# TropComplique/MultiPoseNet

Measured on AMD Instinct MI355X. Metric: images/sec keypoint fwd+bwd+Adam @512x512 bs32/GPU, higher is better.
Workload: dtype bf16; 1 GPU; MobileNet-v1+FPN+keypoint_subnet fwd+bwd+Adam, 512x512, per-GPU batch 32; global_batch=32, parallelism=dp1, hip_graph=True, rccl_ranks=1

## Files before the change

include/mpn.h:

```cpp
#ifndef MPN_H_
#define MPN_H_

#include <stddef.h>
#include <stdint.h>

#ifdef __cplusplus
extern "C" {
#endif

#define MPN_VERSION 600

enum { MPN_F32 = 0, MPN_BF16 = 1, MPN_F16 = 2  };

enum {
    MPN_OK = 0,
    MPN_ERR_BAD_SHAPE = -1,
    MPN_ERR_BAD_DTYPE = -2,
    MPN_ERR_BAD_ALIGN = -3,
    MPN_ERR_HIP = -4,
    MPN_ERR_BAD_ARG = -5,
    MPN_ERR_WORKSPACE = -6,
    MPN_ERR_BAD_DATA = -7
};

// ... 34 lines not shown
                         const float* bn_shift, int bn_act, float* part, mpn_stream_t stream);
int mpn_conv_bwd_data_bn_grouped(int njobs, const void* const* dy, const void* const* w_packed_t, void* const* dx, int N,
                                 const int* H, const int* W, int K, int C, const int* dy_stride, const int* dx_stride,
                                 int dtype, const void* const* bn_x, const int* bn_x_stride, const float* const* bn_scale,
                                 const float* const* bn_shift, int bn_act, float* const* part, mpn_stream_t stream);

int mpn_conv_wgrad_num_parts(int N, int H, int W, int Cin, int Cout, int ksize, int dtype);
int mpn_conv_bwd_weight(const void* x, const void* dy, float* part, int N, int H, int W, int Cin,
                        int Cout, int x_stride, int dy_stride, int ksize, int dtype, const float* in_scale,
                        const float* in_shift, int in_act, mpn_stream_t stream);

int mpn_conv1x1_bwd_fused_supported(int Cin, int Cout, int dtype);
int mpn_conv1x1_bwd_fused(const void* x, const void* dy, const float* w, void* dx, float* wpart, float* bn_part, int N, int H, int W,
                          int Cin, int Cout, int x_stride, int dy_stride, int dx_stride, int dtype, const float* in_scale,
                          const float* in_shift, int in_act, mpn_stream_t stream);
int mpn_conv1x1_bwd_fused_apply_supported(int Cin, int Cout, int dtype);
int mpn_conv1x1_bwd_fused_apply(const void* x, const void* g, const void* y_raw, const float* w, void* dx, float* wpart, float* bn_part,
                                int N, int H, int W, int Cin, int Cout, int x_stride, int g_stride, int y_stride, int dx_stride,
                                int dtype, const float* in_scale, const float* in_shift, int in_act, const float* ap_scale,
                                const float* ap_shift, const float* ap_mean, const float* ap_invstd, const float* ap_k1,
                                const float* ap_k2, int ap_act, mpn_stream_t stream);
int mpn_conv_wgrad_grouped_num_parts(int njobs, int N, const int* H, const int* W, int Cin, int Cout, int ksize, int dtype,
                                     int* nparts);
int mpn_conv_bwd_weight_grouped(int njobs, const void* const* x, const void* const* dy, float* const* part, int N,
                                const int* H, const int* W, int Cin, int Cout, const int* x_stride, const int* dy_stride,
                                int ksize, int dtype, const float* const* in_scale, const float* const* in_shift,
                                int in_act, mpn_stream_t stream);

int mpn_bn_stats_num_parts(long long M);
int mpn_bn_stats(const void* x, long long M, int C, int dtype, float* part, mpn_stream_t stream);
// ... 563 lines not shown
```

multiposenet_amd/_lib.py:

```python
import ctypes
import os

_HERE = os.path.dirname(os.path.abspath(__file__))
LIB_PATH = os.environ.get("MPN_LIB") or os.path.join(_HERE, "libmpn_hip.so")

MPN_VERSION = 600
MPN_F32, MPN_BF16, MPN_F16 = 0, 1, 2
ACT_NONE, ACT_RELU, ACT_RELU6 = 0, 1, 2

_c = ctypes
_P = _c.c_void_p
_I = _c.c_int
_F = _c.c_float
_D = _c.c_double
_Z = _c.c_size_t
_L = _c.c_longlong

SIGNATURES = {
    "mpn_version": (_I, []),
    "mpn_last_error": (_I, [_c.c_char_p, _Z]),
    "mpn_heatmap_decode_workspace_bytes": (_Z, [_I]),
    "mpn_heatmap_decode": (_I, [_P, _I, _I, _I, _I, _I, _P, _F, _P, _P, _P, _P, _Z, _P]),
    "mpn_heatmap_render_workspace_bytes": (_Z, [_I]),
    "mpn_heatmap_render": (_I, [_P, _P, _P, _I, _I, _I, _I, _I, _P, _P, _Z, _P]),
# ... 7 lines not shown
    "mpn_conv_packed_bytes": (_Z, [_I, _I, _I, _I, _I]),
    "mpn_conv_pack_weights": (_I, [_P, _I, _I, _I, _I, _I, _P, _P]),
    "mpn_conv_pack_desc_bytes": (_Z, []),
    "mpn_conv_pack_desc_fill": (_I, [_P, _P, _I, _I, _I, _I, _I, _P, _I]),
    "mpn_conv_pack_weights_batched": (_I, [_P, _I, _I, _I, _P]),
    "mpn_conv_num_parts": (_I, [_I, _I, _I, _I]),
    "mpn_conv_stats_rows": (_I, [_I, _I, _I, _I, _I, _I, _I]),
    "mpn_conv_fwd": (_I, [_P, _P, _P, _I, _I, _I, _I, _I, _I, _I, _I, _I, _P, _P, _I, _P, _P, _P]),
    "mpn_conv_fwd_grouped": (_I, [_I, _P, _P, _P, _I, _P, _P, _I, _I, _P, _P, _I, _I, _P, _P, _I, _P, _P]),
    "mpn_conv_wgrad_num_parts": (_I, [_I, _I, _I, _I, _I, _I, _I]),
    "mpn_conv_bwd_weight": (_I, [_P, _P, _P, _I, _I, _I, _I, _I, _I, _I, _I, _I, _P, _P, _I, _P]),
    "mpn_conv1x1_bwd_fused_supported": (_I, [_I, _I, _I]),
    "mpn_conv1x1_bwd_fused": (_I, [_P, _P, _P, _P, _P, _P, _I, _I, _I, _I, _I, _I, _I, _I, _I, _P, _P, _I, _P]),
    "mpn_conv1x1_bwd_fused_apply_supported": (_I, [_I, _I, _I]),
    "mpn_conv1x1_bwd_fused_apply": (_I, [_P, _P, _P, _P, _P, _P, _P, _I, _I, _I, _I, _I, _I, _I, _I, _I, _I, _P, _P, _I, _P, _P, _P, _P, _P, _P, _I, _P]),
    "mpn_conv_wgrad_grouped_num_parts": (_I, [_I, _I, _P, _P, _I, _I, _I, _I, _P]),
    "mpn_conv_bwd_weight_grouped": (_I, [_I, _P, _P, _P, _I, _P, _P, _I, _I, _P, _P, _I, _I, _P, _P, _I, _P]),
    "mpn_bn_stats_num_parts": (_I, [_L]),
    "mpn_bn_stats": (_I, [_P, _L, _I, _I, _P, _P]),
    "mpn_bn_finalize": (_I, [_P, _I, _I, _L, _P, _P, _P, _P, _F, _F, _P, _P, _P, _P, _P]),
    "mpn_bn_inference_affine": (_I, [_I, _P, _P, _P, _P, _F, _P, _P, _P]),
    "mpn_bn_act_apply": (_I, [_P, _P, _L, _I, _I, _P, _P, _I, _P]),
    "mpn_bn_bwd_reduce": (_I, [_P, _P, _L, _I, _I, _P, _P, _P, _P, _I, _P, _P]),
    "mpn_bn_bwd_finalize": (_I, [_P, _I, _I, _L, _P, _P, _P, _P, _P]),
    "mpn_bn_bwd_apply": (_I, [_P, _P, _L, _I, _I, _P, _P, _P, _P, _P, _P, _I, _P, _P]),
    "mpn_dwconv_out_size": (_I, [_I, _I]),
    "mpn_dwconv_num_parts": (_I, [_I, _I, _I, _I, _I, _I]),
    "mpn_dwconv_fwd": (_I, [_P, _P, _P, _I, _I, _I, _I, _I, _I, _P, _P, _I, _I, _P, _P]),
    "mpn_dwconv_bwd_data": (_I, [_P, _P, _P, _I, _I, _I, _I, _I, _I, _P]),
    "mpn_dwconv_bwd_data_bn_num_parts": (_I, [_I, _I, _I, _I, _I, _I]),
# ... 278 lines not shown
```

multiposenet_amd/csrc/conv_wgrad.hip:

```cpp
#include "common.h"
#include <type_traits>

namespace {

template <typename T> using HT = H16<std::conditional_t<sizeof(T) == 2, T, bf16_t>>;
typedef float f32x4_t __attribute__((ext_vector_type(4)));

constexpr int kThreads = 256;
constexpr int kHaloW = 18, kHaloH = 10;

struct WgradParams {
    const void* x;
    const void* dy;
    float* part;
    const float* in_scale;
    const float* in_shift;
    int in_act;
    int N, H, W, Cin, Cout;
    int xs, dys;
    int tiles_x, tiles_y;
    long long M;
    int ntiles;
    int nsplit;
    int n_cg, n_cb;
// ... 35 lines not shown
template <> __device__ __forceinline__ float round_to_storage<half_t>(float v) { return (float)(_Float16)v; }
template <typename T> __device__ __forceinline__ uint2 pack4_storage(const float (&g)[4]);
template <> __device__ __forceinline__ uint2 pack4_storage<bf16_t>(const float (&g)[4]) {
    return make_uint2(pack_bf16x2(g[0], g[1]), pack_bf16x2(g[2], g[3]));
}
template <> __device__ __forceinline__ uint2 pack4_storage<half_t>(const float (&g)[4]) {
    typedef _Float16 h2_t __attribute__((ext_vector_type(2)));
    const h2_t a = {(_Float16)g[0], (_Float16)g[1]}, b = {(_Float16)g[2], (_Float16)g[3]};
    return make_uint2(__builtin_bit_cast(unsigned, a), __builtin_bit_cast(unsigned, b));
}

template <typename H> __device__ __forceinline__ typename H::x4 tr_read(const unsigned char* base, int off) {
    return H::tr_read(base + off);
}

template <typename T, int TAPS, int RBA, int RBD>
__global__ __launch_bounds__(kThreads, 2) void conv_wgrad_kernel(const WgradParams p) {
    constexpr int ES = (int)sizeof(T);
    constexpr int VE = 16 / ES;
    constexpr int CG = RBA / ES;
    constexpr int BNW = RBD / ES;
    constexpr int DSLOTS = RBD / 16;
    constexpr int NPIXA = TAPS == 9 ? kHaloW * kHaloH : 128;
    constexpr int MT_TOTAL = CG / 16, NT_TOTAL = BNW / 16;
    constexpr int WM = MT_TOTAL >= 2 ? 2 : 1;
    constexpr int WN = 4 / WM;
    constexpr int MTW = MT_TOTAL / WM;
    constexpr int NTW = NT_TOTAL / WN;
    constexpr int KPIX = ES == 2 ? 32 : 4;
    constexpr int KSTEPS = 128 / KPIX;
// ... 264 lines not shown
    for (int c = tid; c < CG; c += NT) {
        const bool ok = affine && ci0 + c < p.Cin;
        aff[c] = ok ? p.in_scale[ci0 + c] : 1.f;
        aff[CG + c] = ok ? p.in_shift[ci0 + c] : 0.f;
    }

    const int aslot = tid % ASLOTS;
    const int dslot = tid % DSLOTS;

    Vec16<T> v[AVEC], dv[DVEC];
    Vec16<T> ev[DAPPLY ? DVEC : 1];
    unsigned inb = 0u, inbd = 0u;
    static_assert(!DAPPLY || DG, "the apply pass folds into the fused thin backward");
    float* apc = reinterpret_cast<float*>(Os + OBYTES + (DG ? 8 * 2 * CG * (int)sizeof(float) : 0));
    float alo = -INFINITY, ahi = INFINITY;
    if constexpr (DAPPLY) {
        for (int c = tid; c < BNW; c += NT) {
            const bool ok = co0 + c < p.Cout;
            const float s_ = ok ? p.ap_scale[co0 + c] : 0.f, h_ = ok ? p.ap_shift[co0 + c] : 0.f, m_ = ok ? p.ap_mean[co0 + c] : 0.f;
            const float i_ = ok ? p.ap_invstd[co0 + c] : 0.f, a_ = ok ? p.ap_k1[co0 + c] : 0.f, b_ = ok ? p.ap_k2[co0 + c] : 0.f;
            apc[c] = s_; apc[BNW + c] = h_;
            apc[2 * BNW + c] = -s_ * b_ * i_;
            apc[3 * BNW + c] = -s_ * (a_ - m_ * i_ * b_);
        }
        alo = (p.ap_act != MPN_ACT_NONE) ? 0.f : -INFINITY;
        ahi = (p.ap_act == MPN_ACT_RELU6) ? 6.f : INFINITY;
    }

    int relA[AVEC], hyx[AVEC], relD[DVEC];
    {
        const int ace = ci0 + aslot * VE, dce = co0 + dslot * VE;
#pragma unroll
        for (int i = 0; i < AVEC; ++i) {
            const int vi = tid + i * NT;
            const int pix = vi / ASLOTS;
            const bool ok = ace < p.Cin && vi < NPIXA * ASLOTS;
            if (TAPS == 9) {
                const int hy = pix / kHaloW, hx = pix - hy * kHaloW;
// ... 41 lines not shown
                unsigned md = 0u;
#pragma unroll
                for (int i = 0; i < DVEC; ++i) md |= ((dvalid && drow0 + i * (NT / DSLOTS) < mleft) ? 1u : 0u) << i;
                inbd = md;
            }
            __builtin_amdgcn_sched_barrier(0);
#pragma unroll
            for (int i = 0; i < AVEC; ++i) {
                const u32x4_t q = __builtin_amdgcn_raw_buffer_load_b128(rsx, (int)(relAb[i] + tbA), 0, 0);
                v[i].raw = make_uint4(q.x, q.y, q.z, q.w);
            }
#pragma unroll
            for (int i = 0; i < DVEC; ++i) {
                const u32x4_t q = __builtin_amdgcn_raw_buffer_load_b128(rsd, (int)(relDb[i] + tbD), 0, 0);
                dv[i].raw = make_uint4(q.x, q.y, q.z, q.w);
            }
            if constexpr (DAPPLY) {
                const unsigned tbE = (unsigned)tile * 128u * (unsigned)p.ap_xs * (unsigned)sizeof(T);
#pragma unroll
                for (int i = 0; i < DVEC; ++i) {
                    const u32x4_t q = __builtin_amdgcn_raw_buffer_load_b128(rse, (int)(relEb[i] + tbE), 0, 0);
                    ev[i].raw = make_uint4(q.x, q.y, q.z, q.w);
                }
            }
            __builtin_amdgcn_sched_barrier(0);
            return;
        }
        int oy0 = 0, ox0 = 0, baseA, baseD, mleft = 0;
        if (TAPS == 9) {
            const int tx = tile % p.tiles_x;
            const int t2 = tile / p.tiles_x;
            const int ty = t2 % p.tiles_y;
            const int img = t2 / p.tiles_y;
            oy0 = ty * 8;
            ox0 = tx * 16;
            const int pix0 = (img * p.H + oy0) * p.W + ox0;
            baseA = pix0 * p.xs;
            baseD = pix0 * p.dys;
// ... 20 lines not shown
        for (int i = 0; i < DVEC; ++i) {
            const int r = drow0 + i * (NT / DSLOTS);
            bool ok = dvalid;
            if (TAPS == 9) ok = ok && oy0 + (r >> 4) < p.H && ox0 + (r & 15) < p.W;
            else ok = ok && r < mleft;
            od[i] = ok ? baseD + relD[i] : 0;
            md |= (ok ? 1u : 0u) << i;
        }
        inb = ma;
        inbd = md;
        __builtin_amdgcn_sched_barrier(0);
#pragma unroll
        for (int i = 0; i < AVEC; ++i) v[i].load(x + oa[i]);
#pragma unroll
        for (int i = 0; i < DVEC; ++i) dv[i].load(dy + od[i]);
        if constexpr (DAPPLY) {
            const T* __restrict__ ax = reinterpret_cast<const T*>(p.ap_x);
#pragma unroll
            for (int i = 0; i < DVEC; ++i) {
                const int r = drow0 + i * (NT / DSLOTS);
                const bool ok = (inbd >> i) & 1u;
                ev[i].load(ax + (ok ? (long long)(tile * 128 + r) * p.ap_xs + co0 + dslot * VE : 0));
            }
        }
        __builtin_amdgcn_sched_barrier(0);
    };

    auto commit_tile = [&](unsigned char* As, unsigned char* Ds) {
        float sc[VE], sh[VE];
        if (affine) {
#pragma unroll
            for (int j = 0; j < VE; j += 4) {
                const float4 a = *reinterpret_cast<const float4*>(aff + aslot * VE + j);
                const float4 c = *reinterpret_cast<const float4*>(aff + CG + aslot * VE + j);
                sc[j] = a.x; sc[j + 1] = a.y; sc[j + 2] = a.z; sc[j + 3] = a.w;
                sh[j] = c.x; sh[j + 1] = c.y; sh[j + 2] = c.z; sh[j + 3] = c.w;
            }
        }
#pragma unroll
        for (int i = 0; i < AVEC; ++i) {
            const int vi = tid + i * NT;
            if (vi < NPIXA * ASLOTS) {
                const int pix = vi / ASLOTS;
// ... 4 lines not shown
#pragma unroll
                    for (int j = 0; j < VE; ++j) f[j] = __builtin_amdgcn_fmed3f(f[j] * sc[j] + sh[j], lo, hi);
                    Vec16<T> o;
                    o.pack(f);
                    q = *reinterpret_cast<const uint4*>(&o.raw);
                }
                if (!BUF && !((inb >> i) & 1u)) q = make_uint4(0u, 0u, 0u, 0u);
                *reinterpret_cast<uint4*>(As + pix * SA + aslot * 16) = q;
                if constexpr (DG) {
                    uint4 r = *reinterpret_cast<const uint4*>(&v[i].raw);
                    if (!BUF && !((inb >> i) & 1u)) r = make_uint4(0u, 0u, 0u, 0u);
                    *reinterpret_cast<uint4*>(Rs + pix * SA + aslot * 16) = r;
                }
            }
        }
#pragma unroll
        for (int i = 0; i < DVEC; ++i) {
            const int r = (tid / DSLOTS) + i * (NT / DSLOTS);
            uint4 q = *reinterpret_cast<const uint4*>(&dv[i].raw);
            if constexpr (DAPPLY) {
                float d[VE], f[VE], asc[VE], ash[VE], acb[VE], acc_[VE];
                dv[i].unpack(d);
                ev[i].unpack(f);
#pragma unroll
                for (int j4 = 0; j4 < VE; j4 += 4) {
                    const f32x4_t q0 = *reinterpret_cast<const f32x4_t*>(apc + dslot * VE + j4), q1 = *reinterpret_cast<const f32x4_t*>(apc + BNW + dslot * VE + j4);
                    const f32x4_t q2 = *reinterpret_cast<const f32x4_t*>(apc + 2 * BNW + dslot * VE + j4), q3 = *reinterpret_cast<const f32x4_t*>(apc + 3 * BNW + dslot * VE + j4);
#pragma unroll
                    for (int j = 0; j < 4; ++j) { asc[j4 + j] = q0[j]; ash[j4 + j] = q1[j]; acb[j4 + j] = q2[j]; acc_[j4 + j] = q3[j]; }
                }
#pragma unroll
                for (int j = 0; j < VE; ++j) {
                    const float pre = f[j] * asc[j] + ash[j];
                    const float gg = (pre > alo && pre < ahi) ? d[j] : 0.f;
                    d[j] = asc[j] * gg + (acb[j] * f[j] + acc_[j]);
                }
                Vec16<T> o;
                o.pack(d);
                q = *reinterpret_cast<const uint4*>(&o.raw);
            }
            if ((!BUF || DAPPLY) && !((inbd >> i) & 1u)) q = make_uint4(0u, 0u, 0u, 0u);
            *reinterpret_cast<uint4*>(Ds + r * SD + dslot * 16) = q;
        }
    };

#ifdef MPN_DIAG
    unsigned long long ph[4] = {0, 0, 0, 0}, t_prev = 0;
#define MPN_WG_STAMP(k) do { if (p.dbg) { const unsigned long long t_ = __builtin_amdgcn_s_memtime(); \
                                          ph[k] += t_ - t_prev; t_prev = t_; } } while (0)
#else
#define MPN_WG_STAMP(k) do { } while (0)
#endif
    const int grp = STAGGER ? wave >> 2 : 0;
    const int ntl = p.ntiles > split ? (p.ntiles - split + p.nsplit - 1) / p.nsplit : 0;
    const int ahead = 1 + grp;
// ... 6 lines not shown
        for (int mt = 0; mt < MTH; ++mt) {
#pragma unroll
            for (int ks = 0; ks < KS2; ++ks) {
                const int ci = ci0 + (dg_mt0 + mt) * 16 + l15, co = co0 + ks * 32 + lq * 8;
                float f[8];
#pragma unroll
                for (int j = 0; j < 8; ++j) f[j] = (ci < p.Cin && co + j < p.Cout) ? p.wf[(long long)ci * p.Cout + co + j] : 0.f;
                Vec16<T> o;
                o.pack(f);
                wfr[mt][ks] = __builtin_bit_cast(X8, o.raw);
            }
#pragma unroll
            for (int r = 0; r < 4; ++r) { bsum[mt][r] = 0.f; bsq[mt][r] = 0.f; }
        }
    }
    if (ntl > 0) load_tile(split);
    __syncthreads();
    if (ntl > 0) commit_tile(smem, smem + NBUF * ABYTES);
    if (grp == 1) {
        if (ntl > 1) load_tile(split + p.nsplit);
        __syncthreads();
        if (ntl > 1) commit_tile(smem + ABYTES, smem + NBUF * ABYTES + DBYTES);
    }
#ifdef MPN_DIAG
    if (p.dbg) t_prev = __builtin_amdgcn_s_memtime();
#endif
#pragma unroll 1
    for (int it = 0; it < ntl; ++it) {
        const int buf = NBUF == 2 ? (it & 1) : 0;
        unsigned char* As = smem + buf * ABYTES;
        unsigned char* Ds = smem + NBUF * ABYTES + buf * DBYTES;
        const bool more = it + ahead < ntl;
        if (more) load_tile(split + (it + ahead) * p.nsplit);
        MPN_WG_STAMP(1);
        __syncthreads();
        MPN_WG_STAMP(2);
        const int qq = l15 >> 2, pp = l15 & 3;
        const unsigned char* a_lane = As + (4 * lq + qq) * SA + pp * 8 + mt0 * 32;
        const unsigned char* d_lane = Ds + (4 * lq + qq) * SD + pp * 8 + nt0 * 32;
        constexpr int STEPS = TAPS * MTW;
        constexpr int TOTAL = 4 * STEPS;
        constexpr int RING0 = NTW >= 4 ? 4 : ((TAPS == 9 && RBA == 256) ? 4 : 6);
        constexpr int RING = RING0 < STEPS ? RING0 : STEPS;
        constexpr int KSA = (TAPS == 9 ? 2 * kHaloW : 32) * SA, KSD = 32 * SD;
        auto a_load = [&](int gs) -> X8 {
            const int ks = gs / STEPS, step = gs % STEPS;
            const int t = step / MTW, i = step % MTW;
            const int row = TAPS == 9 ? (t / 3) * kHaloW + (t % 3) : 0;
// ... 17 lines not shown
#pragma unroll
        for (int gs = 0; gs < TOTAL; ++gs) {
            const int ks = gs / STEPS, step = gs % STEPS;
            if (step == STEPS - RING && ks + 1 < 4) {
#pragma unroll
                for (int j = 0; j < NTW; ++j) bfr[(ks + 1) & 1][j] = b_load(ks + 1, j);
            }
            if (gs + RING - 1 < TOTAL) ar[(gs + RING - 1) % RING] = a_load(gs + RING - 1);
            const int t = step / MTW, i = step % MTW;
#pragma unroll
            for (int j = 0; j < NTW; ++j)
                acc[t][i][j] = H::mfma(ar[gs % RING], bfr[ks & 1][j], acc[t][i][j]);
            __builtin_amdgcn_sched_barrier(0);
        }
        if constexpr (DG) {
            const bool bnr = p.bn_part != nullptr;
#pragma unroll 1
            for (int j = 0; j < DGS; ++j) {
                const int px = (dg_pt0 + j) * 16 + l15;
                f32x4_t dacc[MTH];
#pragma unroll
                for (int mt = 0; mt < MTH; ++mt) dacc[mt] = (f32x4_t){0.f, 0.f, 0.f, 0.f};
#pragma unroll
                for (int ks = 0; ks < KS2; ++ks) {
                    const X8 dfr = *reinterpret_cast<const X8*>(Ds + px * SD + ks * 64 + lq * 16);
#pragma unroll
                    for (int mt = 0; mt < MTH; ++mt) dacc[mt] = H::mfma(wfr[mt][ks], dfr, dacc[mt]);
                }
#pragma unroll
                for (int mt = 0; mt < MTH; ++mt) {
// ... 9 lines not shown
                        const float pre = xf[r] * sc4[r] + sh4[r];
                        const float d = round_to_storage<T>(dacc[mt][r]);
                        g[r] = (!bnr || (pre > lo && pre < hi)) ? d : 0.f;
                        bsum[mt][r] += g[r];
                        bsq[mt][r] += g[r] * xf[r];
                    }
                    *reinterpret_cast<uint2*>(Os + px * OS + cl * 2) = pack4_storage<T>(g);
                }
            }
        }
        MPN_WG_STAMP(3);
        __syncthreads();
        MPN_WG_STAMP(2);
        if (more) {
            const int nb = NBUF == 2 ? ((it + ahead) & 1) : 0;
            commit_tile(smem + nb * ABYTES, smem + NBUF * ABYTES + nb * DBYTES);
        }
        if constexpr (DG) {
            const int tile = split + it * p.nsplit;
            const int mleft = (int)(p.M - (long long)tile * 128);
            T* __restrict__ dxp = reinterpret_cast<T*>(p.dx) + (long long)tile * 128 * p.dxs + ci0;
            for (int v0 = tid; v0 < 128 * ASLOTS; v0 += NT) {
                const int pr = v0 / ASLOTS, sl = v0 - pr * ASLOTS;
                if (pr < mleft && ci0 + sl * 8 < p.Cin)
                    *reinterpret_cast<uint4*>(dxp + (long long)pr * p.dxs + sl * 8) = *reinterpret_cast<const uint4*>(Os + pr * OS + sl * 16);
            }
        }
        MPN_WG_STAMP(0);
    }
    if (STAGGER && grp == 0) __syncthreads();
#ifdef MPN_DIAG
// ... 314 lines not shown
    for (int j = 0; j < njobs; ++j)
        if (int rc = wgrad_fill_job(grp.p[j], who, x[j], dy[j], part[j], N, H[j], W[j], Cin, Cout, x_stride ? x_stride[j] : 0,
                                    dy_stride ? dy_stride[j] : 0, ksize, 2, in_scale[j], in_shift[j], in_act, geoms[j], nsplit[j]))
            return rc;
    const int blocks = wgrad_group_lay(grp, njobs);
    hipStream_t st = (hipStream_t)stream;
    if (dtype == MPN_F16) return wgrad16_dispatch(Cin, Cout, ksize, [&](auto geo) { return launch_wgrad_bf16_grouped<half_t>(geo, grp, blocks, st); });
    return wgrad16_dispatch(Cin, Cout, ksize, [&](auto geo) { return launch_wgrad_bf16_grouped<bf16_t>(geo, grp, blocks, st); });
}

namespace {
template <typename T, int RBA, int RBD, int WM, bool DAPPLY = false>
int launch_conv1x1_bwd_fused(const WgradParams& p, hipStream_t st) {
    constexpr int CG = RBA / 2;
    constexpr int smem = 128 * (RBA + 32) + 128 * (RBD + 32) + 2 * CG * (int)sizeof(float) + 128 * (RBA + 32) + 128 * (RBA + 16) +
                         8 * 2 * CG * (int)sizeof(float) + (DAPPLY ? 4 * (RBD / 2) * (int)sizeof(float) : 0);
    static_assert(smem <= 160 * 1024, "LDS budget");
    static mpn_attr_mask_t attr_mask{0};
    MPN_HIP(mpn_ensure_dynamic_lds((const void*)conv1x1_bwd_fused_kernel<T, RBA, RBD, WM, DAPPLY>, smem, &attr_mask));
    conv1x1_bwd_fused_kernel<T, RBA, RBD, WM, DAPPLY><<<dim3((unsigned)p.nsplit), dim3(512), smem, st>>>(p);
    MPN_LAUNCH_CHECK();
    return MPN_OK;
}
}

extern "C" int mpn_conv1x1_bwd_fused_supported(int Cin, int Cout, int dtype) {
    return (dtype == MPN_BF16 && Cin > 0 && Cout > 0 && Cin % 8 == 0 && Cout % 8 == 0 && Cin <= 128 && Cout <= 128) ? 1 : 0;
}

namespace {
struct Conv1x1Apply { const void* y_raw; int y_stride; const float *scale, *shift, *mean, *invstd, *k1, *k2; int act; };
int conv1x1_bwd_fused_impl(const void* x, const void* dy, const float* w, void* dx, float* wpart, float* bn_part, int N, int H,
                           int W, int Cin, int Cout, int x_stride, int dy_stride, int dx_stride, int dtype,
                           const float* in_scale, const float* in_shift, int in_act, const Conv1x1Apply* ap, mpn_stream_t stream) {
    const char* who = ap ? "conv1x1_bwd_fused_apply" : "conv1x1_bwd_fused";
    MPN_REQUIRE(mpn_conv1x1_bwd_fused_supported(Cin, Cout, dtype), MPN_ERR_BAD_SHAPE, "%s: layer not covered (Cin %d, Cout %d)", who, Cin, Cout);
    MPN_REQUIRE(w && dx && in_scale && in_shift, MPN_ERR_BAD_ARG, "%s: null pointer", who);
    MPN_REQUIRE(bn_part != nullptr || ap == nullptr, MPN_ERR_BAD_ARG, "%s: needs the reduction's slab", who);
    MPN_REQUIRE(mpn_aligned16(dx), MPN_ERR_BAD_ALIGN, "%s: pointers must be 16-byte aligned", who);
    MPN_REQUIRE(dx != x && dx != dy, MPN_ERR_BAD_ARG, "%s: dx must not alias an input", who);
    const WgradGeom g = wgrad_geom(N, H, W, Cin, Cout, 1, 2);
    MPN_REQUIRE(g.n_cg == 1 && g.n_cb == 1, MPN_ERR_BAD_SHAPE, "%s: one block tile must hold the layer", who);
    WgradParams p;
    if (int rc = wgrad_fill_job(p, who, x, dy, wpart, N, H, W, Cin, Cout, x_stride, dy_stride, 1, 2, in_scale, in_shift, in_act, g, g.nsplit))
        return rc;
    p.wf = w; p.dx = dx; p.bn_part = bn_part; p.dxs = dx_stride > 0 ? dx_stride : Cin;
    MPN_REQUIRE(p.dxs >= Cin && p.dxs % 8 == 0, MPN_ERR_BAD_SHAPE, "%s: dx's pixel stride must be a multiple of 8 not below Cin", who);
    hipStream_t st = (hipStream_t)stream;
    const bool thin32 = Cin <= 32 && Cout <= 64, wide = Cin > 64;
    if (ap != nullptr) {
        MPN_REQUIRE(!wide, MPN_ERR_BAD_SHAPE, "conv1x1_bwd_fused_apply: layer not covered (Cin %d, Cout %d)", Cin, Cout);
        MPN_REQUIRE(ap->y_raw && ap->scale && ap->shift && ap->mean && ap->invstd && ap->k1 && ap->k2 && mpn_aligned16(ap->y_raw), MPN_ERR_BAD_ARG,
                    "conv1x1_bwd_fused_apply: bad batch-norm arguments");
        p.ap_x = ap->y_raw; p.ap_xs = ap->y_stride > 0 ? ap->y_stride : Cout;
        MPN_REQUIRE(p.ap_xs >= Cout && p.ap_xs % 8 == 0 && (long long)N * H * W * p.ap_xs < (1ll << 31), MPN_ERR_BAD_SHAPE, "conv1x1_bwd_fused_apply: bad raw-output stride");
        p.ap_scale = ap->scale; p.ap_shift = ap->shift; p.ap_mean = ap->mean; p.ap_invstd = ap->invstd; p.ap_k1 = ap->k1; p.ap_k2 = ap->k2; p.ap_act = ap->act;
        return thin32 ? launch_conv1x1_bwd_fused<bf16_t, 64, 128, 2, true>(p, st) : launch_conv1x1_bwd_fused<bf16_t, 128, 256, 2, true>(p, st);
    }
    if (wide) return launch_conv1x1_bwd_fused<bf16_t, 256, 256, 4>(p, st);
    return thin32 ? launch_conv1x1_bwd_fused<bf16_t, 64, 128, 2>(p, st) : launch_conv1x1_bwd_fused<bf16_t, 128, 256, 2>(p, st);
}
}

extern "C" int mpn_conv1x1_bwd_fused(const void* x, const void* dy, const float* w, void* dx, float* wpart, float* bn_part, int N, int H,
                                     int W, int Cin, int Cout, int x_stride, int dy_stride, int dx_stride, int dtype,
                                     const float* in_scale, const float* in_shift, int in_act, mpn_stream_t stream) {
    return conv1x1_bwd_fused_impl(x, dy, w, dx, wpart, bn_part, N, H, W, Cin, Cout, x_stride, dy_stride, dx_stride, dtype, in_scale, in_shift,
                                  in_act, nullptr, stream);
}

extern "C" int mpn_conv1x1_bwd_fused_apply_supported(int Cin, int Cout, int dtype) {
    return (mpn_conv1x1_bwd_fused_supported(Cin, Cout, dtype) && Cin <= 64) ? 1 : 0;
}

extern "C" int mpn_conv1x1_bwd_fused_apply(const void* x, const void* g, const void* y_raw, const float* w, void* dx, float* wpart,
                                           float* bn_part, int N, int H, int W, int Cin, int Cout, int x_stride, int g_stride, int y_stride,
                                           int dx_stride, int dtype, const float* in_scale, const float* in_shift, int in_act,
                                           const float* ap_scale, const float* ap_shift, const float* ap_mean, const float* ap_invstd,
                                           const float* ap_k1, const float* ap_k2, int ap_act, mpn_stream_t stream) {
    const Conv1x1Apply ap = {y_raw, y_stride, ap_scale, ap_shift, ap_mean, ap_invstd, ap_k1, ap_k2, ap_act};
    return conv1x1_bwd_fused_impl(x, g, w, dx, wpart, bn_part, N, H, W, Cin, Cout, x_stride, g_stride, dx_stride, dtype, in_scale, in_shift,
                                  in_act, &ap, stream);
}
```

multiposenet_amd/net.py:

```python
import math
import os
from collections import OrderedDict

import numpy as np
import torch

from . import _lib, ops
from ._lib import ACT_NONE, ACT_RELU, ACT_RELU6
from .model_state import ModelState, _Arena, is_trainable, resolve_device

NUM_KEYPOINTS = 17
DOWNSAMPLE = 4
DIVISOR = 128
DEPTH = 128
STRIDES_AND_FILTERS = [(1, 64), (2, 128), (1, 128), (2, 256), (1, 256), (2, 512), (1, 512), (1, 512),
                       (1, 512), (1, 512), (1, 512), (2, 1024), (1, 1024)]
FEATURE_BLOCKS = {3: "c2", 5: "c3", 11: "c4", 13: "c5"}


def depth(x, depth_multiplier):
    return max(int(x * depth_multiplier), 8)


def variable_shapes(depth_multiplier=1.0):
# ... 550 lines not shown

    def _dw_walks_fused(self, b, g, i):
        s, (N, _, _, C) = self.blocks[i]["stride"], b["dw"][i].shape
        return (self.fuse_dw_bn and (s == 2 or self._dw_lateral(g, i) is None)
                and ops.dwconv_bwd_fused_supported(N, *b["hw"][i], C, s, self.dtype))

    def _dw_folds_apply(self, b, g, i):
        s, (N, _, _, C) = self.blocks[i]["stride"], b["dw"][i].shape
        return (self.fuse_dw_apply and self._dw_walks_fused(b, g, i)
                and ops.dwconv_bwd_fused_apply_supported(N, *b["hw"][i], C, s, self.dtype))

    def _backward_pointwise(self, b, g, sp, slab, i, dA, reduced, raw, fold=False):
        blk = self.blocks[i]
        pw, x, dY = blk["pw"], b["dw"][i], g["dw"][i]
        fused = self.fuse_conv_bn and ops.conv1x1_bwd_fused_supported(pw.cin, pw.cout, self.dtype) and pw.cin <= 64
        apply = fused and ops.conv1x1_bwd_fused_apply_supported(pw.cin, pw.cout, self.dtype)
        ops.bn_backward(blk["pw_bn"], dA, b["pw"][i], sp, reduced_parts=reduced, raw=raw, apply=not apply)
        rows = 0
        with _lib.tagged("pointwise"):
            if fused:
                rows = ops.conv1x1_bwd_fused(x, dA, pw.w, blk["dw_bn"], dY, slab[id(pw.dw)], sp,
                                             apply_bn=blk["pw_bn"] if apply else None, y_raw=b["pw"][i] if apply else None)
            else:
                ops.conv_bwd_weight(x, dA, 1, blk["dw_bn"].affine, pw.dw, slab[id(pw.dw)], reduce=False)
                if self.fuse_conv_bn and ops.conv_bwd_data_bn_supported(pw.cout, pw.cin, 1, self.dtype):
                    rows = ops.conv_bwd_data_bn(dA, pw.packed.bwd, pw.cin, 1, blk["dw_bn"], x, dY, sp)
                else:
                    ops.conv_fwd(dA, pw.packed.bwd, pw.cin, 1, None, out=dY)
        applied = not (fold and rows > 0)
        ops.bn_backward(blk["dw_bn"], dY, x, sp, reduced_parts=rows, raw=True, apply=applied)
        return dY, applied
# ... 40 lines not shown
```

multiposenet_amd/ops.py:

```python
import ctypes
from collections import namedtuple

import torch

from . import _lib
from ._lib import ACT_NONE, ACT_RELU, ACT_RELU6, call, ptr, stream_ptr

BN_MOMENTUM = 0.95
BN_EPSILON = 1e-3

LAUNCH_JOBS_ALONE = False

Affine = namedtuple("Affine", ["scale", "shift", "act"])


def _f32(n, dev):
    return torch.empty(n, dtype=torch.float32, device=dev)


def _check_nhwc(x, name="x"):
    if x.dim() != 4 or not x.is_contiguous():
        raise ValueError(f"{name} must be a contiguous NHWC tensor, got shape {tuple(x.shape)}")
    if x.dtype not in (torch.float32, torch.bfloat16):
        raise ValueError(f"{name}: unsupported dtype {x.dtype}")
# ... 116 lines not shown
         _arr([t.shape[2] for t in dys], ctypes.c_int), k, int(c), _arr([_slice_stride(t, k) for t in dys], ctypes.c_int),
         _arr([_slice_stride(o, c) for o in outs], ctypes.c_int), _lib.dtype_code(dys[0].dtype), _arr(xs_bn),
         _arr([_slice_stride(x, c) for x in xs_bn], ctypes.c_int), _arr([b.scale for b in bns]), _arr([b.shift for b in bns]),
         int(bns[0].act), _arr(parts), stream_ptr())
    return [conv_stats_rows(N, t.shape[1], t.shape[2], k, c, 3, t.dtype) for t in dys]


def conv1x1_bwd_fused_supported(cin, cout, dtype):
    return _lib.lib().mpn_conv1x1_bwd_fused_supported(int(cin), int(cout), _lib.dtype_code(dtype)) == 1


def conv1x1_bwd_fused_apply_supported(cin, cout, dtype):
    return _lib.lib().mpn_conv1x1_bwd_fused_apply_supported(int(cin), int(cout), _lib.dtype_code(dtype)) == 1


def conv1x1_bwd_fused(x, dy, w, bn, out, wpart, bn_part, apply_bn=None, y_raw=None):
    N, H, W, cin = x.shape
    cout = dy.shape[3]
    rows = conv_wgrad_num_parts(N, H, W, cin, cout, 1, x.dtype)
    if wpart.numel() < rows * cin * cout or (bn_part is not None and bn_part.numel() < rows * 2 * cin):
        raise ValueError("conv1x1_bwd_fused: partial slab too small")
    if apply_bn is not None:
        a = apply_bn
        call("mpn_conv1x1_bwd_fused_apply", ptr(x), ptr(dy), ptr(y_raw), ptr(w), ptr(out), ptr(wpart), ptr(bn_part), N, H, W, cin, cout,
             _slice_stride(x, cin), _slice_stride(dy, cout), _slice_stride(y_raw, cout), _slice_stride(out, cin), _lib.dtype_code(x.dtype),
             ptr(bn.scale), ptr(bn.shift), int(bn.act), ptr(a.scale), ptr(a.shift), ptr(a.mean), ptr(a.invstd), ptr(a.k1), ptr(a.k2),
             int(a.act), stream_ptr())
        return rows
    call("mpn_conv1x1_bwd_fused", ptr(x), ptr(dy), ptr(w), ptr(out), ptr(wpart), ptr(bn_part), N, H, W, cin, cout, _slice_stride(x, cin),
         _slice_stride(dy, cout), _slice_stride(out, cin), _lib.dtype_code(x.dtype), ptr(bn.scale), ptr(bn.shift), int(bn.act), stream_ptr())
    return rows


def conv_wgrad_num_parts(N, H, W, cin, cout, ksize, dtype):
    return _lib.lib().mpn_conv_wgrad_num_parts(N, H, W, cin, cout, ksize, _lib.dtype_code(dtype))


def conv_bwd_weight(x, dy, ksize, affine, dw_out, part=None, reduce=True):
    N, H, W, cin = x.shape
# ... 607 lines not shown
```

Before: 4466 images/s.

## Extend fused BN-apply into 1x1 backward for wide layers and defer raw loads

Adds an apply128 entry point that lets the fused 1x1 backward kernel also perform the batch-norm backward apply for wider layers (Cin up to 128), using the 256x256 tile variant. The raw-output loads are split into a separate load_raw step that can be issued late, after the MFMA work, when there are enough tiles. The apply math moves into the commit stage with an exact-rounding path that mimics the unfused ordering. The aim is to remove a separate BN apply pass over memory for these layers, at the cost of more LDS, more registers and a complicated numerics-matching path. However, net.py still gates fusion on pw.cin <= 64, so the wide path may never run.

```diff
diff --git a/include/mpn.h b/include/mpn.h
--- a/include/mpn.h
+++ b/include/mpn.h
@@ -72,6 +72,12 @@
 int mpn_conv1x1_bwd_fused(const void* x, const void* dy, const float* w, void* dx, float* wpart, float* bn_part, int N, int H, int W,
                           int Cin, int Cout, int x_stride, int dy_stride, int dx_stride, int dtype, const float* in_scale,
                           const float* in_shift, int in_act, mpn_stream_t stream);
+int mpn_conv1x1_bwd_fused_apply128_supported(int Cin, int Cout, int dtype);
+int mpn_conv1x1_bwd_fused_apply128(const void* x, const void* g, const void* y_raw, const float* w, void* dx, float* wpart, float* bn_part,
+                                   int N, int H, int W, int Cin, int Cout, int x_stride, int g_stride, int y_stride, int dx_stride,
+                                   int dtype, const float* in_scale, const float* in_shift, int in_act, const float* ap_scale,
+                                   const float* ap_shift, const float* ap_mean, const float* ap_invstd, const float* ap_k1,
+                                   const float* ap_k2, int ap_act, mpn_stream_t stream);
 int mpn_conv1x1_bwd_fused_apply_supported(int Cin, int Cout, int dtype);
 int mpn_conv1x1_bwd_fused_apply(const void* x, const void* g, const void* y_raw, const float* w, void* dx, float* wpart, float* bn_part,
                                 int N, int H, int W, int Cin, int Cout, int x_stride, int g_stride, int y_stride, int dx_stride,
diff --git a/multiposenet_amd/_lib.py b/multiposenet_amd/_lib.py
--- a/multiposenet_amd/_lib.py
+++ b/multiposenet_amd/_lib.py
@@ -45,6 +45,8 @@
     "mpn_conv1x1_bwd_fused": (_I, [_P, _P, _P, _P, _P, _P, _I, _I, _I, _I, _I, _I, _I, _I, _I, _P, _P, _I, _P]),
     "mpn_conv1x1_bwd_fused_apply_supported": (_I, [_I, _I, _I]),
     "mpn_conv1x1_bwd_fused_apply": (_I, [_P, _P, _P, _P, _P, _P, _P, _I, _I, _I, _I, _I, _I, _I, _I, _I, _I, _P, _P, _I, _P, _P, _P, _P, _P, _P, _I, _P]),
+    "mpn_conv1x1_bwd_fused_apply128_supported": (_I, [_I, _I, _I]),
+    "mpn_conv1x1_bwd_fused_apply128": (_I, [_P, _P, _P, _P, _P, _P, _P, _I, _I, _I, _I, _I, _I, _I, _I, _I, _I, _P, _P, _I, _P, _P, _P, _P, _P, _P, _I, _P]),
     "mpn_conv_wgrad_grouped_num_parts": (_I, [_I, _I, _P, _P, _I, _I, _I, _I, _P]),
     "mpn_conv_bwd_weight_grouped": (_I, [_I, _P, _P, _P, _I, _P, _P, _I, _I, _P, _P, _I, _I, _P, _P, _I, _P]),
     "mpn_bn_stats_num_parts": (_I, [_L]),
diff --git a/multiposenet_amd/csrc/conv_wgrad.hip b/multiposenet_amd/csrc/conv_wgrad.hip
--- a/multiposenet_amd/csrc/conv_wgrad.hip
+++ b/multiposenet_amd/csrc/conv_wgrad.hip
@@ -73,6 +73,31 @@
     return H::tr_read(base + off);
 }
 
+template <typename T>
+__device__ __forceinline__ uint2 bn_apply_staged4(uint2 graw, uint2 yraw, const f32x4_t (&q)[6], bool generic, bool unfused67, float lo, float hi) {
+#pragma clang fp contract(off)
+    Raw4h<T> gr, yr;
+    gr.v = graw; yr.v = yraw;
+    float g[4], y[4];
+    raw4_unpack(gr, g);
+    raw4_unpack(yr, y);
+#pragma unroll
+    for (int j = 0; j < 4; ++j) {
+        const float pre = __builtin_fmaf(y[j], q[0][j], q[1][j]);
+        const float gg = (pre > lo && pre < hi) ? g[j] : 0.f;
+        if (generic) {
+            const float xhat = (y[j] - q[2][j]) * q[3][j];
+            g[j] = q[0][j] * __builtin_fmaf(-xhat, q[5][j], gg - q[4][j]);
+        } else {
+            const float t = q[2][j] * y[j], u = q[0][j] * gg;
+            const float plain = (q[3][j] + t) + u;
+            const float nested = __builtin_fmaf(q[0][j], gg, __builtin_fmaf(q[2][j], y[j], q[3][j]));
+            g[j] = (j >= 2 && unfused67) ? plain : nested;
+        }
+    }
+    return pack4_storage<T>(g);
+}
+
 template <typename T, int TAPS, int RBA, int RBD>
 __global__ __launch_bounds__(kThreads, 2) void conv_wgrad_kernel(const WgradParams p) {
     constexpr int ES = (int)sizeof(T);
@@ -367,14 +392,16 @@
     static_assert(!DAPPLY || DG, "the apply pass folds into the fused thin backward");
     float* apc = reinterpret_cast<float*>(Os + OBYTES + (DG ? 8 * 2 * CG * (int)sizeof(float) : 0));
     float alo = -INFINITY, ahi = INFINITY;
+    const bool apgen = DAPPLY && 256 % (p.Cout / VE) != 0;
     if constexpr (DAPPLY) {
         for (int c = tid; c < BNW; c += NT) {
             const bool ok = co0 + c < p.Cout;
             const float s_ = ok ? p.ap_scale[co0 + c] : 0.f, h_ = ok ? p.ap_shift[co0 + c] : 0.f, m_ = ok ? p.ap_mean[co0 + c] : 0.f;
             const float i_ = ok ? p.ap_invstd[co0 + c] : 0.f, a_ = ok ? p.ap_k1[co0 + c] : 0.f, b_ = ok ? p.ap_k2[co0 + c] : 0.f;
             apc[c] = s_; apc[BNW + c] = h_;
-            apc[2 * BNW + c] = -s_ * b_ * i_;
-            apc[3 * BNW + c] = -s_ * (a_ - m_ * i_ * b_);
+            apc[2 * BNW + c] = apgen ? m_ : (-s_ * b_) * i_;
+            apc[3 * BNW + c] = apgen ? i_ : -s_ * __builtin_fmaf(-(m_ * i_), b_, a_);
+            apc[4 * BNW + c] = a_; apc[5 * BNW + c] = b_;
         }
         alo = (p.ap_act != MPN_ACT_NONE) ? 0.f : -INFINITY;
         ahi = (p.ap_act == MPN_ACT_RELU6) ? 6.f : INFINITY;
@@ -446,14 +473,6 @@
             for (int i = 0; i < DVEC; ++i) {
                 const u32x4_t q = __builtin_amdgcn_raw_buffer_load_b128(rsd, (int)(relDb[i] + tbD), 0, 0);
                 dv[i].raw = make_uint4(q.x, q.y, q.z, q.w);
-            }
-            if constexpr (DAPPLY) {
-                const unsigned tbE = (unsigned)tile * 128u * (unsigned)p.ap_xs * (unsigned)sizeof(T);
-#pragma unroll
-                for (int i = 0; i < DVEC; ++i) {
-                    const u32x4_t q = __builtin_amdgcn_raw_buffer_load_b128(rse, (int)(relEb[i] + tbE), 0, 0);
-                    ev[i].raw = make_uint4(q.x, q.y, q.z, q.w);
-                }
             }
             __builtin_amdgcn_sched_barrier(0);
             return;
@@ -504,19 +523,24 @@
         for (int i = 0; i < AVEC; ++i) v[i].load(x + oa[i]);
 #pragma unroll
         for (int i = 0; i < DVEC; ++i) dv[i].load(dy + od[i]);
-        if constexpr (DAPPLY) {
-            const T* __restrict__ ax = reinterpret_cast<const T*>(p.ap_x);
-#pragma unroll
-            for (int i = 0; i < DVEC; ++i) {
-                const int r = drow0 + i * (NT / DSLOTS);
-                const bool ok = (inbd >> i) & 1u;
-                ev[i].load(ax + (ok ? (long long)(tile * 128 + r) * p.ap_xs + co0 + dslot * VE : 0));
-            }
-        }
         __builtin_amdgcn_sched_barrier(0);
     };
-
-    auto commit_tile = [&](unsigned char* As, unsigned char* Ds) {
+    constexpr bool LATE_RAW = DAPPLY && MT_TOTAL >= 8;
+    auto load_raw = [&](int tile) {
+        if constexpr (DAPPLY) {
+            static_assert(!DAPPLY || BUF, "the apply pass folds into the 1x1 kernel");
+            const unsigned tbE = (unsigned)tile * 128u * (unsigned)p.ap_xs * (unsigned)sizeof(T);
+            __builtin_amdgcn_sched_barrier(0);
+#pragma unroll
+            for (int i = 0; i < DVEC; ++i) {
+                const u32x4_t q = __builtin_amdgcn_raw_buffer_load_b128(rse, (int)(relEb[i] + tbE), 0, 0);
+                ev[i].raw = make_uint4(q.x, q.y, q.z, q.w);
+            }
+            __builtin_amdgcn_sched_barrier(0);
+        }
+    };
+
+    auto commit_tile = [&](unsigned char* As, unsigned char* Ds, int tile) {
         float sc[VE], sh[VE];
         if (affine) {
 #pragma unroll
@@ -551,31 +575,31 @@
                 }
             }
         }
+        if constexpr (DAPPLY) {
+            const unsigned vec0 = (unsigned)tile * 128u * (unsigned)(p.Cout / VE) + (unsigned)((co0 >> 3) + dslot);
+#pragma unroll
+            for (int h = 0; h < 2; ++h) {
+                const float* c4 = apc + dslot * VE + h * 4;
+                f32x4_t q[6];
+#pragma unroll
+                for (int k = 0; k < 4; ++k) q[k] = *reinterpret_cast<const f32x4_t*>(c4 + k * BNW);
+                q[4] = q[5] = (f32x4_t){0.f, 0.f, 0.f, 0.f};
+                if (apgen) { q[4] = *reinterpret_cast<const f32x4_t*>(c4 + 4 * BNW); q[5] = *reinterpret_cast<const f32x4_t*>(c4 + 5 * BNW); }
+#pragma unroll
+                for (int i = 0; i < DVEC; ++i) {
+                    const unsigned vec = vec0 + (unsigned)(drow0 + i * (NT / DSLOTS)) * (unsigned)(p.Cout / VE);
+                    const bool unf = h == 1 && ((vec >> 8) & 3u) != 2u;
+                    const uint2 gq = h ? make_uint2(dv[i].raw.z, dv[i].raw.w) : make_uint2(dv[i].raw.x, dv[i].raw.y);
+                    const uint2 yq = h ? make_uint2(ev[i].raw.z, ev[i].raw.w) : make_uint2(ev[i].raw.x, ev[i].raw.y);
+                    const uint2 o = bn_apply_staged4<T>(gq, yq, q, apgen, unf, alo, ahi);
+                    if (h) { dv[i].raw.z = o.x; dv[i].raw.w = o.y; } else { dv[i].raw.x = o.x; dv[i].raw.y = o.y; }
+                }
+            }
+        }
 #pragma unroll
         for (int i = 0; i < DVEC; ++i) {
             const int r = (tid / DSLOTS) + i * (NT / DSLOTS);
             uint4 q = *reinterpret_cast<const uint4*>(&dv[i].raw);
-            if constexpr (DAPPLY) {
-                float d[VE], f[VE], asc[VE], ash[VE], acb[VE], acc_[VE];
-                dv[i].unpack(d);
-                ev[i].unpack(f);
-#pragma unroll
-                for (int j4 = 0; j4 < VE; j4 += 4) {
-                    const f32x4_t q0 = *reinterpret_cast<const f32x4_t*>(apc + dslot * VE + j4), q1 = *reinterpret_cast<const f32x4_t*>(apc + BNW + dslot * VE + j4);
-                    const f32x4_t q2 = *reinterpret_cast<const f32x4_t*>(apc + 2 * BNW + dslot * VE + j4), q3 = *reinterpret_cast<const f32x4_t*>(apc + 3 * BNW + dslot * VE + j4);
-#pragma unroll
-                    for (int j = 0; j < 4; ++j) { asc[j4 + j] = q0[j]; ash[j4 + j] = q1[j]; acb[j4 + j] = q2[j]; acc_[j4 + j] = q3[j]; }
-                }
-#pragma unroll
-                for (int j = 0; j < VE; ++j) {
-                    const float pre = f[j] * asc[j] + ash[j];
-                    const float gg = (pre > alo && pre < ahi) ? d[j] : 0.f;
-                    d[j] = asc[j] * gg + (acb[j] * f[j] + acc_[j]);
-                }
-                Vec16<T> o;
-                o.pack(d);
-                q = *reinterpret_cast<const uint4*>(&o.raw);
-            }
             if ((!BUF || DAPPLY) && !((inbd >> i) & 1u)) q = make_uint4(0u, 0u, 0u, 0u);
             *reinterpret_cast<uint4*>(Ds + r * SD + dslot * 16) = q;
         }
@@ -612,13 +636,13 @@
             for (int r = 0; r < 4; ++r) { bsum[mt][r] = 0.f; bsq[mt][r] = 0.f; }
         }
     }
-    if (ntl > 0) load_tile(split);
+    if (ntl > 0) { load_tile(split); load_raw(split); }
     __syncthreads();
-    if (ntl > 0) commit_tile(smem, smem + NBUF * ABYTES);
+    if (ntl > 0) commit_tile(smem, smem + NBUF * ABYTES, split);
     if (grp == 1) {
         if (ntl > 1) load_tile(split + p.nsplit);
         __syncthreads();
-        if (ntl > 1) commit_tile(smem + ABYTES, smem + NBUF * ABYTES + DBYTES);
+        if (ntl > 1) commit_tile(smem + ABYTES, smem + NBUF * ABYTES + DBYTES, split + p.nsplit);
     }
 #ifdef MPN_DIAG
     if (p.dbg) t_prev = __builtin_amdgcn_s_memtime();
@@ -629,7 +653,10 @@
         unsigned char* As = smem + buf * ABYTES;
         unsigned char* Ds = smem + NBUF * ABYTES + buf * DBYTES;
         const bool more = it + ahead < ntl;
-        if (more) load_tile(split + (it + ahead) * p.nsplit);
+        if (more) {
+            load_tile(split + (it + ahead) * p.nsplit);
+            if (!LATE_RAW) load_raw(split + (it + ahead) * p.nsplit);
+        }
         MPN_WG_STAMP(1);
         __syncthreads();
         MPN_WG_STAMP(2);
@@ -677,6 +704,7 @@
             __builtin_amdgcn_sched_barrier(0);
         }
         if constexpr (DG) {
+            if (LATE_RAW && more) load_raw(split + (it + ahead) * p.nsplit);
             const bool bnr = p.bn_part != nullptr;
 #pragma unroll 1
             for (int j = 0; j < DGS; ++j) {
@@ -716,7 +744,7 @@
         MPN_WG_STAMP(2);
         if (more) {
             const int nb = NBUF == 2 ? ((it + ahead) & 1) : 0;
-            commit_tile(smem + nb * ABYTES, smem + NBUF * ABYTES + nb * DBYTES);
+            commit_tile(smem + nb * ABYTES, smem + NBUF * ABYTES + nb * DBYTES, split + (it + ahead) * p.nsplit);
         }
         if constexpr (DG) {
             const int tile = split + it * p.nsplit;
@@ -1061,7 +1089,7 @@
 int launch_conv1x1_bwd_fused(const WgradParams& p, hipStream_t st) {
     constexpr int CG = RBA / 2;
     constexpr int smem = 128 * (RBA + 32) + 128 * (RBD + 32) + 2 * CG * (int)sizeof(float) + 128 * (RBA + 32) + 128 * (RBA + 16) +
-                         8 * 2 * CG * (int)sizeof(float) + (DAPPLY ? 4 * (RBD / 2) * (int)sizeof(float) : 0);
+                         8 * 2 * CG * (int)sizeof(float) + (DAPPLY ? 6 * (RBD / 2) * (int)sizeof(float) : 0);
     static_assert(smem <= 160 * 1024, "LDS budget");
     static mpn_attr_mask_t attr_mask{0};
     MPN_HIP(mpn_ensure_dynamic_lds((const void*)conv1x1_bwd_fused_kernel<T, RBA, RBD, WM, DAPPLY>, smem, &attr_mask));
@@ -1076,12 +1104,13 @@
 }
 
 namespace {
-struct Conv1x1Apply { const void* y_raw; int y_stride; const float *scale, *shift, *mean, *invstd, *k1, *k2; int act; };
+struct Conv1x1Apply { const void* y_raw; int y_stride; const float *scale, *shift, *mean, *invstd, *k1, *k2; int act; int max_cin; };
 int conv1x1_bwd_fused_impl(const void* x, const void* dy, const float* w, void* dx, float* wpart, float* bn_part, int N, int H,
                            int W, int Cin, int Cout, int x_stride, int dy_stride, int dx_stride, int dtype,
                            const float* in_scale, const float* in_shift, int in_act, const Conv1x1Apply* ap, mpn_stream_t stream) {
     const char* who = ap ? "conv1x1_bwd_fused_apply" : "conv1x1_bwd_fused";
     MPN_REQUIRE(mpn_conv1x1_bwd_fused_supported(Cin, Cout, dtype), MPN_ERR_BAD_SHAPE, "%s: layer not covered (Cin %d, Cout %d)", who, Cin, Cout);
+    MPN_REQUIRE(ap == nullptr || Cin <= ap->max_cin, MPN_ERR_BAD_SHAPE, "%s: layer not covered (Cin %d, Cout %d)", who, Cin, Cout);
     MPN_REQUIRE(w && dx && in_scale && in_shift, MPN_ERR_BAD_ARG, "%s: null pointer", who);
     MPN_REQUIRE(bn_part != nullptr || ap == nullptr, MPN_ERR_BAD_ARG, "%s: needs the reduction's slab", who);
     MPN_REQUIRE(mpn_aligned16(dx), MPN_ERR_BAD_ALIGN, "%s: pointers must be 16-byte aligned", who);
@@ -1096,12 +1125,12 @@
     hipStream_t st = (hipStream_t)stream;
     const bool thin32 = Cin <= 32 && Cout <= 64, wide = Cin > 64;
     if (ap != nullptr) {
-        MPN_REQUIRE(!wide, MPN_ERR_BAD_SHAPE, "conv1x1_bwd_fused_apply: layer not covered (Cin %d, Cout %d)", Cin, Cout);
         MPN_REQUIRE(ap->y_raw && ap->scale && ap->shift && ap->mean && ap->invstd && ap->k1 && ap->k2 && mpn_aligned16(ap->y_raw), MPN_ERR_BAD_ARG,
                     "conv1x1_bwd_fused_apply: bad batch-norm arguments");
         p.ap_x = ap->y_raw; p.ap_xs = ap->y_stride > 0 ? ap->y_stride : Cout;
         MPN_REQUIRE(p.ap_xs >= Cout && p.ap_xs % 8 == 0 && (long long)N * H * W * p.ap_xs < (1ll << 31), MPN_ERR_BAD_SHAPE, "conv1x1_bwd_fused_apply: bad raw-output stride");
         p.ap_scale = ap->scale; p.ap_shift = ap->shift; p.ap_mean = ap->mean; p.ap_invstd = ap->invstd; p.ap_k1 = ap->k1; p.ap_k2 = ap->k2; p.ap_act = ap->act;
+        if (wide) return launch_conv1x1_bwd_fused<bf16_t, 256, 256, 4, true>(p, st);
         return thin32 ? launch_conv1x1_bwd_fused<bf16_t, 64, 128, 2, true>(p, st) : launch_conv1x1_bwd_fused<bf16_t, 128, 256, 2, true>(p, st);
     }
     if (wide) return launch_conv1x1_bwd_fused<bf16_t, 256, 256, 4>(p, st);
@@ -1125,7 +1154,20 @@
                                            int dx_stride, int dtype, const float* in_scale, const float* in_shift, int in_act,
                                            const float* ap_scale, const float* ap_shift, const float* ap_mean, const float* ap_invstd,
                                            const float* ap_k1, const float* ap_k2, int ap_act, mpn_stream_t stream) {
-    const Conv1x1Apply ap = {y_raw, y_stride, ap_scale, ap_shift, ap_mean, ap_invstd, ap_k1, ap_k2, ap_act};
+    const Conv1x1Apply ap = {y_raw, y_stride, ap_scale, ap_shift, ap_mean, ap_invstd, ap_k1, ap_k2, ap_act, 64};
     return conv1x1_bwd_fused_impl(x, g, w, dx, wpart, bn_part, N, H, W, Cin, Cout, x_stride, g_stride, dx_stride, dtype, in_scale, in_shift,
                                   in_act, &ap, stream);
 }
+
+extern "C" int mpn_conv1x1_bwd_fused_apply128_supported(int Cin, int Cout, int dtype) {
+    return mpn_conv1x1_bwd_fused_supported(Cin, Cout, dtype);
+}
+extern "C" int mpn_conv1x1_bwd_fused_apply128(const void* x, const void* g, const void* y_raw, const float* w, void* dx, float* wpart,
+                                              float* bn_part, int N, int H, int W, int Cin, int Cout, int x_stride, int g_stride, int y_stride,
+                                              int dx_stride, int dtype, const float* in_scale, const float* in_shift, int in_act,
+                                              const float* ap_scale, const float* ap_shift, const float* ap_mean, const float* ap_invstd,
+                                              const float* ap_k1, const float* ap_k2, int ap_act, mpn_stream_t stream) {
+    const Conv1x1Apply ap = {y_raw, y_stride, ap_scale, ap_shift, ap_mean, ap_invstd, ap_k1, ap_k2, ap_act, 128};
+    return conv1x1_bwd_fused_impl(x, g, w, dx, wpart, bn_part, N, H, W, Cin, Cout, x_stride, g_stride, dx_stride, dtype, in_scale, in_shift,
+                                  in_act, &ap, stream);
+}
diff --git a/multiposenet_amd/net.py b/multiposenet_amd/net.py
--- a/multiposenet_amd/net.py
+++ b/multiposenet_amd/net.py
@@ -588,7 +588,7 @@
         blk = self.blocks[i]
         pw, x, dY = blk["pw"], b["dw"][i], g["dw"][i]
         fused = self.fuse_conv_bn and ops.conv1x1_bwd_fused_supported(pw.cin, pw.cout, self.dtype) and pw.cin <= 64
-        apply = fused and ops.conv1x1_bwd_fused_apply_supported(pw.cin, pw.cout, self.dtype)
+        apply = fused and ops.conv1x1_bwd_fused_apply128_supported(pw.cin, pw.cout, self.dtype)
         ops.bn_backward(blk["pw_bn"], dA, b["pw"][i], sp, reduced_parts=reduced, raw=raw, apply=not apply)
         rows = 0
         with _lib.tagged("pointwise"):
diff --git a/multiposenet_amd/ops.py b/multiposenet_amd/ops.py
--- a/multiposenet_amd/ops.py
+++ b/multiposenet_amd/ops.py
@@ -154,6 +154,10 @@
     return _lib.lib().mpn_conv1x1_bwd_fused_apply_supported(int(cin), int(cout), _lib.dtype_code(dtype)) == 1
 
 
+def conv1x1_bwd_fused_apply128_supported(cin, cout, dtype):
+    return _lib.lib().mpn_conv1x1_bwd_fused_apply128_supported(int(cin), int(cout), _lib.dtype_code(dtype)) == 1
+
+
 def conv1x1_bwd_fused(x, dy, w, bn, out, wpart, bn_part, apply_bn=None, y_raw=None):
     N, H, W, cin = x.shape
     cout = dy.shape[3]
@@ -162,7 +166,7 @@
         raise ValueError("conv1x1_bwd_fused: partial slab too small")
     if apply_bn is not None:
         a = apply_bn
-        call("mpn_conv1x1_bwd_fused_apply", ptr(x), ptr(dy), ptr(y_raw), ptr(w), ptr(out), ptr(wpart), ptr(bn_part), N, H, W, cin, cout,
+        call("mpn_conv1x1_bwd_fused_apply128", ptr(x), ptr(dy), ptr(y_raw), ptr(w), ptr(out), ptr(wpart), ptr(bn_part), N, H, W, cin, cout,
              _slice_stride(x, cin), _slice_stride(dy, cout), _slice_stride(y_raw, cout), _slice_stride(out, cin), _lib.dtype_code(x.dtype),
              ptr(bn.scale), ptr(bn.shift), int(bn.act), ptr(a.scale), ptr(a.shift), ptr(a.mean), ptr(a.invstd), ptr(a.k1), ptr(a.k2),
              int(a.act), stream_ptr())
```

Result: no change. 4428 images/s (-0.8%).
